# mx-mark/VideoTransformer-pytorch

Hardware: NVIDIA H100
Metric: clips/sec (BxTx3x224x224) TimeSformer-B fwd+bwd (higher is better)
Workload: dtype bf16

## Files before the change

videotransformer_pytorch_b200/csrc/vt_gemm.cu:

```cuda
#include <stdlib.h>
#include <string.h>

#include "vt_common.cuh"
#include "vt_sm90.cuh"

namespace vt {

constexpr int BM = 128;
constexpr int BK = 64;
constexpr int GEMM_THREADS = 384;
constexpr int CHUNK_BYTES = 64 * BK * 2;

struct GemmDev {
  int M, N, K;
  int kblocks, splits;
  int num_m, num_n, tiles;
  int epi;
  const float* bias;
  const float* bias2;
  void* out;
  const void* aux;
  long long ldo, ldaux;
  const int* out_row;
  const int* aux_row;
  const float* row_scale;
  long long split_stride;
  int map_period, map_skip, map_tcount;
  long long map_stride_t, map_stride_p, map_stride_b, map_base;
  float* special_out;
  long long special_ld;
  const float* a_scale;
  const float* b_scale;
};

constexpr int EPI_BOX_BYTES = 64 * 64 * 2;
constexpr int SE_F32 = 3;

template <int BN, int SE>
struct GemmCfg {
  static constexpr int A_BYTES = BM * BK * 2;
  static constexpr int B_BYTES = BN * BK * 2;
  static constexpr int STAGE_BYTES = A_BYTES + B_BYTES;
  static constexpr int EPI_TILE_BYTES = BM * BN * 2;
  static constexpr int F32_PITCH = BN + 8;
  static constexpr int EPI_BYTES = SE == SE_F32 ? BM * F32_PITCH * 4 : SE == 1 ? EPI_TILE_BYTES : 0;
  static constexpr int SMEM_LIMIT = 232448, SMEM_EXTRA = 1024  + 256 ;
  static constexpr int STAGES_FIT = (SMEM_LIMIT - SMEM_EXTRA - EPI_BYTES) / STAGE_BYTES;
  static constexpr int STAGES = STAGES_FIT < 6 ? STAGES_FIT : 6;
  static constexpr int SMEM_BYTES = STAGES * STAGE_BYTES + EPI_BYTES + SMEM_EXTRA;
  static_assert(STAGES >= 2 && SMEM_BYTES <= SMEM_LIMIT, "shared memory budget");
};

template <int BN, int TA, int TB>
__device__ __forceinline__ void wgmma_tile(float (&acc)[BN / 2], uint64_t da, uint64_t db, uint32_t scale_d) {
  if constexpr (BN == 256) wgmma_m64n256k16<TA, TB>(acc, da, db, scale_d);
  else if constexpr (BN == 192) wgmma_m64n192k16<TA, TB>(acc, da, db, scale_d);
  else wgmma_m64n128k16<TA, TB>(acc, da, db, scale_d);
}

struct EpiRow {
  char* out;
  const char* aux;
  float s;
};

__device__ __forceinline__ EpiRow epi_row(const GemmDev& p, int row, int split) {
  EpiRow r{nullptr, nullptr, 1.0f};
  if (row >= p.M) return r;
  if (p.row_scale) r.s = p.row_scale[row];
  if (p.epi == VT_EPI_F32) {
    float* out = static_cast<float*>(p.out);
    const float* aux = static_cast<const float*>(p.aux);
    if (p.map_period > 0) {
      const int outer = row / p.map_period, inner = row - outer * p.map_period;
      if (inner < p.map_skip) {
        if (p.special_out) r.out = reinterpret_cast<char*>(p.special_out + (long long)outer * p.special_ld);
        return r;
      }
      const long long off = p.map_base + (long long)(outer % p.map_tcount) * p.map_stride_t +
                            (long long)(inner - p.map_skip) * p.map_stride_p + (long long)(outer / p.map_tcount) * p.map_stride_b;
      r.out = reinterpret_cast<char*>(out + off);
      r.aux = reinterpret_cast<const char*>(aux + off);
      return r;
    }
    const int orow = p.out_row ? p.out_row[row] : row;
    if (orow >= 0) r.out = reinterpret_cast<char*>(out + (long long)split * p.split_stride + (long long)orow * p.ldo);
    if (aux) {
      const int arow = p.aux_row ? p.aux_row[row] : row;
      if (arow >= 0) r.aux = reinterpret_cast<const char*>(aux + (long long)arow * p.ldaux);
    }
    return r;
  }
  const int orow = p.out_row ? p.out_row[row] : row;
  if (orow < 0) return r;
  r.out = reinterpret_cast<char*>(static_cast<__nv_bfloat16*>(p.out) + (long long)orow * p.ldo);
  return r;
}

__device__ __forceinline__ void add_bias(const GemmDev& p, int n, float& v0, float& v1) {
  if (p.bias) {
    const float2 b = __ldg(reinterpret_cast<const float2*>(p.bias + n));
    v0 += b.x; v1 += b.y;
  }
}
__device__ __forceinline__ uint32_t gelu_pair(uint32_t z) {
  const float2 zr = unpack_bf16x2(z);
  return pack_bf16x2(gelu_fast(zr.x), gelu_fast(zr.y));
}

__device__ __forceinline__ void epi_pair(const GemmDev& p, const EpiRow& r, int n, float v0, float v1) {
  if (!r.out) return;
  add_bias(p, n, v0, v1);
  if (p.epi == VT_EPI_BF16) {
    *reinterpret_cast<uint32_t*>(reinterpret_cast<__nv_bfloat16*>(r.out) + n) = pack_bf16x2(r.s * v0, r.s * v1);
  } else if (p.epi == VT_EPI_F32) {
    float2 a = make_float2(0.f, 0.f);
    if (r.aux) a = *reinterpret_cast<const float2*>(reinterpret_cast<const float*>(r.aux) + n);
    if (p.bias2) {
      const float2 b2 = __ldg(reinterpret_cast<const float2*>(p.bias2 + n));
      a.x += b2.x; a.y += b2.y;
    }
    *reinterpret_cast<float2*>(reinterpret_cast<float*>(r.out) + n) = make_float2(fmaf(r.s, v0, a.x), fmaf(r.s, v1, a.y));
  } else {
    *reinterpret_cast<uint32_t*>(reinterpret_cast<__nv_bfloat16*>(r.out) + n) = gelu_pair(pack_bf16x2(r.s * v0, r.s * v1));
  }
}

template <int BN, int EPI>
__device__ __forceinline__ void epi_stage(const GemmDev& p, const float (&acc)[BN / 2], uint8_t* stage, int row0, int n0,
                                          int warp, int lane) {
  const int r = warp * 16 + (lane >> 2);
  float s[2] = {1.0f, 1.0f};
  if (p.row_scale) {
#pragma unroll
    for (int h = 0; h < 2; ++h)
      if (row0 + r + 8 * h < p.M) s[h] = p.row_scale[row0 + r + 8 * h];
  }
  const uint32_t a1 = smem_u32(stage) + r * 128 + 4 * (lane & 3) + ((lane >> 2) << 4);
#pragma unroll
  for (int j = 0; j < BN / 8; ++j) {
    const int n = n0 + 8 * j + 2 * (lane & 3);
    if (n >= p.N) break;
#pragma unroll
    for (int h = 0; h < 2; ++h) {
      const uint32_t off = (j >> 3) * EPI_BOX_BYTES + h * 8 * 128;
      const uint32_t o = (a1 ^ ((j & 7) << 4)) + off;
      float v0 = acc[4 * j + 2 * h], v1 = acc[4 * j + 2 * h + 1];
      add_bias(p, n, v0, v1);
      if (EPI == VT_EPI_BF16) st_shared_u32(o, pack_bf16x2(s[h] * v0, s[h] * v1));
      else st_shared_u32(o, gelu_pair(pack_bf16x2(s[h] * v0, s[h] * v1)));
    }
  }
}

struct Tile {
  int m0, n0, split, kb0, kb1;
};

template <int BN>
__device__ __forceinline__ Tile tile_at(const GemmDev& p, int t) {
  Tile c;
  const int nt = t % p.num_n, rest = t / p.num_n;
  const int mt = rest % p.num_m;
  c.split = rest / p.num_m;
  c.m0 = mt * BM;
  c.n0 = nt * BN;
  c.kb0 = (int)(((long long)p.kblocks * c.split) / p.splits);
  c.kb1 = (int)(((long long)p.kblocks * (c.split + 1)) / p.splits);
  return c;
}

template <int BN>
__device__ __forceinline__ void epi_f32_io(const GemmDev& p, float* stage, uint64_t* full, uint64_t* ready, int half, int lane) {
  constexpr int PITCH = GemmCfg<BN, SE_F32>::F32_PITCH;
  uint32_t tj = 0;
  for (int t = blockIdx.x; t < p.tiles; t += gridDim.x, ++tj) {
    const Tile c = tile_at<BN>(p, t);
    const int cols = p.N - c.n0 < BN ? p.N - c.n0 : BN;
    const uint32_t bytes = (uint32_t)cols * 4;
    const int row0 = c.m0 + half * 64 + lane;
    const EpiRow e0 = epi_row(p, row0, c.split), e1 = epi_row(p, row0 + 32, c.split);
    float* s0 = stage + lane * PITCH;
    float* s1 = s0 + 32 * PITCH;
    tma_store_wait_read_all();
    uint32_t tx = 0;
    if (p.aux) {
      if (e0.out && e0.aux) tx += bytes;
      if (e1.out && e1.aux) tx += bytes;
      for (int h = 0; h < 2; ++h) {
        const EpiRow& e = h ? e1 : e0;
        if (e.out && !e.aux)
          for (int i = 0; i < cols; i += 4) st_shared_zero16(smem_u32((h ? s1 : s0) + i));
      }
    }
    mbar_arrive_expect_tx(full, tx);
    if (tx) {
      if (e0.out && e0.aux) bulk_load_1d(s0, reinterpret_cast<const float*>(e0.aux) + c.n0, bytes, full);
      if (e1.out && e1.aux) bulk_load_1d(s1, reinterpret_cast<const float*>(e1.aux) + c.n0, bytes, full);
    }
    mbar_wait(ready, tj & 1);
    if (e0.out) bulk_store_1d(reinterpret_cast<float*>(e0.out) + c.n0, s0, bytes);
    if (e1.out) bulk_store_1d(reinterpret_cast<float*>(e1.out) + c.n0, s1, bytes);
    tma_store_commit();
  }
  tma_store_wait_read_all();
}

template <int BN>
__device__ __forceinline__ void epi_f32_stage(const GemmDev& p, const float (&acc)[BN / 2], const float* stage, int row0, int n0,
                                              int warp, int lane) {
  constexpr int PITCH = GemmCfg<BN, SE_F32>::F32_PITCH;
  const int r = warp * 16 + (lane >> 2);
  float s[2] = {1.0f, 1.0f};
  if (p.row_scale) {
#pragma unroll
    for (int h = 0; h < 2; ++h)
      if (row0 + r + 8 * h < p.M) s[h] = p.row_scale[row0 + r + 8 * h];
  }
  const uint32_t a0 = smem_u32(stage + r * PITCH + 2 * (lane & 3));
#pragma unroll
  for (int j = 0; j < BN / 8; ++j) {
    const int n = n0 + 8 * j + 2 * (lane & 3);
    if (n >= p.N) break;
#pragma unroll
    for (int h = 0; h < 2; ++h) {
      const uint32_t o = a0 + (h * 8 * PITCH + 8 * j) * 4;
      float v0 = acc[4 * j + 2 * h], v1 = acc[4 * j + 2 * h + 1];
      add_bias(p, n, v0, v1);
      float2 a = make_float2(0.f, 0.f);
      if (p.aux) a = ld_shared_f32x2(o);
      if (p.bias2) {
        const float2 b2 = __ldg(reinterpret_cast<const float2*>(p.bias2 + n));
        a.x += b2.x; a.y += b2.y;
      }
      st_shared_f32x2(o, fmaf(s[h], v0, a.x), fmaf(s[h], v1, a.y));
    }
  }
}

template <int BN, int TA, int TB, int SE, int F8>
__device__ __forceinline__ void gemm_wgmma_body(const CUtensorMap& tmA, const CUtensorMap& tmB, const CUtensorMap& tmC,
                                                const GemmDev& p) {
  using Cfg = GemmCfg<BN, SE>;
  static_assert(SE == 0 || SE == 1 || SE == SE_F32, "epilogue kinds: register, staged bf16, staged fp32");
  static_assert(!F8 || (BN == 128 && !TA && !TB), "e4m3 forms: BN = 128, K-major operands");
  static_assert(SE != SE_F32 || BN != 256, "the fp32 staging tile leaves too few ring stages at BN = 256");
  constexpr int STAGES = Cfg::STAGES;
  constexpr int KB_ELEMS = F8 ? 128 : BK;
  constexpr int HALF_BYTES = Cfg::EPI_TILE_BYTES / 2;
  extern __shared__ uint8_t smem_raw[];
  uint8_t* smem = reinterpret_cast<uint8_t*>((reinterpret_cast<uintptr_t>(smem_raw) + 1023) & ~uintptr_t(1023));
  uint8_t* epi_smem = smem + STAGES * Cfg::STAGE_BYTES;
  uint64_t* full_bar = reinterpret_cast<uint64_t*>(epi_smem + Cfg::EPI_BYTES);
  uint64_t* empty_bar = full_bar + STAGES;
  uint64_t* rows_full_bar = empty_bar + STAGES;
  uint64_t* rows_ready_bar = rows_full_bar + 2;

  const int wg = threadIdx.x >> 7;
  if (threadIdx.x == 0) {
    tma_prefetch_desc(&tmA);
    tma_prefetch_desc(&tmB);
    if (SE == 1) tma_prefetch_desc(&tmC);
    for (int i = 0; i < STAGES; ++i) {
      mbar_init(&full_bar[i], 1);
      mbar_init(&empty_bar[i], 8);
    }
    for (int h = 0; h < 2; ++h) {
      mbar_init(&rows_full_bar[h], 32);
      mbar_init(&rows_ready_bar[h], 128);
    }
    fence_barrier_init();
  }
  __syncthreads();

  if (wg == 0) {
    setmaxnreg_dec<40>();
    const int pw = threadIdx.x >> 5;
    if constexpr (SE == SE_F32) {
      if (pw == 1 || pw == 2) {
        float* rows = reinterpret_cast<float*>(epi_smem) + (pw - 1) * 64 * Cfg::F32_PITCH;
        epi_f32_io<BN>(p, rows, &rows_full_bar[pw - 1], &rows_ready_bar[pw - 1], pw - 1, threadIdx.x & 31);
      }
    }
    if (threadIdx.x == 0) {
      uint32_t it = 0;
      uint32_t tj = 0;
      for (int t = blockIdx.x; t < p.tiles; t += gridDim.x, ++tj) {
        const Tile c = tile_at<BN>(p, t);
        for (int kb = c.kb0; kb < c.kb1; ++kb, ++it) {
          const int stage = (int)(it % STAGES);
          mbar_wait(&empty_bar[stage], ((it / STAGES) & 1) ^ 1);
          uint8_t* sA = smem + stage * Cfg::STAGE_BYTES;
          uint8_t* sB = sA + Cfg::A_BYTES;
          mbar_arrive_expect_tx(&full_bar[stage], Cfg::STAGE_BYTES);
          if (!TA) {
            tma_load_2d(sA, &tmA, &full_bar[stage], kb * KB_ELEMS, c.m0);
          } else {
#pragma unroll
            for (int ch = 0; ch < BM / 64; ++ch) tma_load_2d(sA + ch * CHUNK_BYTES, &tmA, &full_bar[stage], c.m0 + ch * 64, kb * BK);
          }
          if (!TB) {
            tma_load_2d(sB, &tmB, &full_bar[stage], kb * KB_ELEMS, c.n0);
          } else {
#pragma unroll
            for (int ch = 0; ch < BN / 64; ++ch) tma_load_2d(sB + ch * CHUNK_BYTES, &tmB, &full_bar[stage], c.n0 + ch * 64, kb * BK);
          }
        }
      }
    }
    return;
  }

  setmaxnreg_inc<232>();
  const int cw = wg - 1;
  const int warp = (threadIdx.x >> 5) & 3, lane = threadIdx.x & 31;
  const bool leader = (threadIdx.x & 127) == 0;
  uint8_t* stage = epi_smem + cw * HALF_BYTES;
  uint32_t it = 0, tj = 0;
  float part[F8 ? BN / 2 : 1];
#pragma unroll
  for (int i = 0; i < (F8 ? BN / 2 : 1); ++i) part[i] = 0.f;
  for (int t = blockIdx.x; t < p.tiles; t += gridDim.x, ++tj) {
    const Tile c = tile_at<BN>(p, t);
    float acc[BN / 2];
#pragma unroll
    for (int i = 0; i < BN / 2; ++i) acc[i] = 0.f;
    if constexpr (F8) {
      for (int kb = c.kb0; kb < c.kb1; ++kb, ++it) {
        const int stage = (int)(it % STAGES);
        mbar_wait(&full_bar[stage], (it / STAGES) & 1);
        const uint32_t a_addr = smem_u32(smem + stage * Cfg::STAGE_BYTES) + cw * 64 * 128;
        const uint32_t b_addr = smem_u32(smem + stage * Cfg::STAGE_BYTES + Cfg::A_BYTES);
        wgmma_fence();
#pragma unroll
        for (int k = 0; k < 4; ++k)
          wgmma_m64n128k32_e4m3(part, sdesc_kmajor(a_addr + k * 32), sdesc_kmajor(b_addr + k * 32), k > 0 ? 1u : 0u);
        wgmma_commit();
        wgmma_wait<0>();
        if (lane == 0) mbar_arrive(&empty_bar[stage]);
#pragma unroll
        for (int i = 0; i < BN / 2; ++i) acc[i] += part[i];
      }
      const int rr = c.m0 + cw * 64 + warp * 16 + (lane >> 2);
      const float sa0 = rr < p.M ? p.a_scale[rr] : 0.f, sa1 = rr + 8 < p.M ? p.a_scale[rr + 8] : 0.f;
#pragma unroll
      for (int j = 0; j < BN / 8; ++j) {
        const int n = c.n0 + 8 * j + 2 * (lane & 3);
        if (n >= p.N) break;
        const float2 sb = __ldg(reinterpret_cast<const float2*>(p.b_scale + n));
        acc[4 * j] *= sa0 * sb.x;
        acc[4 * j + 1] *= sa0 * sb.y;
        acc[4 * j + 2] *= sa1 * sb.x;
        acc[4 * j + 3] *= sa1 * sb.y;
      }
    } else {
    int prev = -1;
    for (int kb = c.kb0; kb < c.kb1; ++kb, ++it) {
      const int stage = (int)(it % STAGES);
      mbar_wait(&full_bar[stage], (it / STAGES) & 1);
      const uint32_t a_addr = smem_u32(smem + stage * Cfg::STAGE_BYTES) + cw * (TA ? CHUNK_BYTES : 64 * 128);
      const uint32_t b_addr = smem_u32(smem + stage * Cfg::STAGE_BYTES + Cfg::A_BYTES);
      wgmma_fence();
#pragma unroll
      for (int k = 0; k < BK / 16; ++k) {
        const uint64_t da = TA ? sdesc_mnmajor(a_addr + k * 2048, CHUNK_BYTES) : sdesc_kmajor(a_addr + k * 32);
        const uint64_t db = TB ? sdesc_mnmajor(b_addr + k * 2048, CHUNK_BYTES) : sdesc_kmajor(b_addr + k * 32);
        wgmma_tile<BN, TA, TB>(acc, da, db, (kb > c.kb0 || k > 0) ? 1u : 0u);
      }
      wgmma_commit();
      wgmma_wait<1>();
      if (prev >= 0 && lane == 0) mbar_arrive(&empty_bar[prev]);
      prev = stage;
    }
    wgmma_wait<0>();
    if (lane == 0) mbar_arrive(&empty_bar[prev]);
    }

    if constexpr (SE == SE_F32) {
      const float* rows = reinterpret_cast<const float*>(epi_smem) + cw * 64 * Cfg::F32_PITCH;
      mbar_wait(&rows_full_bar[cw], tj & 1);
      epi_f32_stage<BN>(p, acc, rows, c.m0 + cw * 64, c.n0, warp, lane);
      fence_proxy_async_smem();
      mbar_arrive(&rows_ready_bar[cw]);
    } else if constexpr (SE == 1) {
      const int row0 = c.m0 + cw * 64;
      if (leader) tma_store_wait_read_all();
      named_bar_sync(1 + cw, 128);
      if (p.epi == VT_EPI_GELU_H) epi_stage<BN, VT_EPI_GELU_H>(p, acc, stage, row0, c.n0, warp, lane);
      else epi_stage<BN, VT_EPI_BF16>(p, acc, stage, row0, c.n0, warp, lane);
      fence_proxy_async_smem();
      named_bar_sync(1 + cw, 128);
      if (leader) {
        if (row0 < p.M) {
#pragma unroll
          for (int b = 0; b < BN / 64; ++b) {
            if (c.n0 + 64 * b >= p.N) break;
            tma_store_2d(&tmC, stage + b * EPI_BOX_BYTES, c.n0 + 64 * b, row0);
          }
        }
        tma_store_commit();
      }
    } else {
      const int r0 = c.m0 + cw * 64 + warp * 16 + (lane >> 2);
      const EpiRow e0 = epi_row(p, r0, c.split), e1 = epi_row(p, r0 + 8, c.split);
#pragma unroll
      for (int j = 0; j < BN / 8; ++j) {
        const int n = c.n0 + 8 * j + 2 * (lane & 3);
        if (n >= p.N) break;
        epi_pair(p, e0, n, acc[4 * j], acc[4 * j + 1]);
        epi_pair(p, e1, n, acc[4 * j + 2], acc[4 * j + 3]);
      }
    }
  }
  if (SE == 1 && leader) tma_store_wait_read_all();
}

template <int BN, int TA, int TB, int SE>
__global__ void __launch_bounds__(GEMM_THREADS, 1)
gemm_wgmma_kernel(const __grid_constant__ CUtensorMap tmA, const __grid_constant__ CUtensorMap tmB,
                  const __grid_constant__ CUtensorMap tmC, const GemmDev p) {
  gemm_wgmma_body<BN, TA, TB, SE, 0>(tmA, tmB, tmC, p);
}

template <int BN, int TA, int TB>
__global__ void __launch_bounds__(GEMM_THREADS, 1)
gemm_f32_kernel(const __grid_constant__ CUtensorMap tmA, const __grid_constant__ CUtensorMap tmB,
                const __grid_constant__ CUtensorMap tmC, const GemmDev p) {
  gemm_wgmma_body<BN, TA, TB, SE_F32, 0>(tmA, tmB, tmC, p);
}

template <int SE>
__global__ void __launch_bounds__(GEMM_THREADS, 1)
gemm_e4m3_kernel(const __grid_constant__ CUtensorMap tmA, const __grid_constant__ CUtensorMap tmB,
                 const __grid_constant__ CUtensorMap tmC, const GemmDev p) {
  gemm_wgmma_body<128, 0, 0, SE, 1>(tmA, tmB, tmC, p);
}

typedef CUresult (*EncodeTiledFn)(CUtensorMap*, CUtensorMapDataType, cuuint32_t, void*, const cuuint64_t*,
                                  const cuuint64_t*, const cuuint32_t*, const cuuint32_t*, CUtensorMapInterleave,
                                  CUtensorMapSwizzle, CUtensorMapL2promotion, CUtensorMapFloatOOBfill);

static EncodeTiledFn get_encode_fn() {
  static EncodeTiledFn fn = nullptr;
  if (!fn) {
    void* ptr = nullptr;
    cudaDriverEntryPointQueryResult qres;
    cudaError_t e = cudaGetDriverEntryPoint("cuTensorMapEncodeTiled", &ptr, cudaEnableDefault, &qres);
    if (e != cudaSuccess || qres != cudaDriverEntryPointSuccess || !ptr) return nullptr;
    fn = reinterpret_cast<EncodeTiledFn>(ptr);
  }
  return fn;
}

static int make_tmap_2d(CUtensorMap* map, int esize, const void* base, long long rows, long long cols, long long ld,
                        int box_rows) {
  EncodeTiledFn fn = get_encode_fn();
  VT_REQUIRE(fn != nullptr, "cuTensorMapEncodeTiled entry point unavailable");
  VT_REQUIRE((reinterpret_cast<uintptr_t>(base) & 15) == 0, "TMA base pointer must be 16-byte aligned");
  VT_REQUIRE((ld * esize) % 16 == 0, "TMA leading dimension must be a multiple of %d elements (got %lld)", 16 / esize, ld);
  cuuint64_t gdim[2] = {(cuuint64_t)cols, (cuuint64_t)rows};
  cuuint64_t gstr[1] = {(cuuint64_t)(ld * esize)};
  cuuint32_t box[2] = {(cuuint32_t)(128 / esize), (cuuint32_t)box_rows};
  cuuint32_t estr[2] = {1u, 1u};
  CUresult r = fn(map, esize == 2 ? CU_TENSOR_MAP_DATA_TYPE_BFLOAT16 : CU_TENSOR_MAP_DATA_TYPE_UINT8, 2, const_cast<void*>(base),
                  gdim, gstr, box, estr,
                  CU_TENSOR_MAP_INTERLEAVE_NONE, CU_TENSOR_MAP_SWIZZLE_128B, CU_TENSOR_MAP_L2_PROMOTION_L2_256B,
                  CU_TENSOR_MAP_FLOAT_OOB_FILL_NONE);
  VT_REQUIRE(r == CUDA_SUCCESS, "cuTensorMapEncodeTiled failed (%d) rows=%lld cols=%lld ld=%lld box_rows=%d", (int)r,
             rows, cols, ld, box_rows);
  return 0;
}

int make_tmap_bf16_2d(CUtensorMap* map, const void* base, long long rows, long long cols, long long ld, int box_rows) {
  return make_tmap_2d(map, 2, base, rows, cols, ld, box_rows);
}

__global__ void reduce_rows_kernel(const float* __restrict__ in, float* __restrict__ out, long long stride, int S,
                                   long long n4, int accumulate, float scale) {
  for (long long i = blockIdx.x * (long long)blockDim.x + threadIdx.x; i < n4; i += (long long)gridDim.x * blockDim.x) {
    float4 acc = make_float4(0.f, 0.f, 0.f, 0.f);
    for (int s = 0; s < S; ++s) {
      const float4 v = *reinterpret_cast<const float4*>(in + (long long)s * stride + i * 4);
      acc.x += v.x; acc.y += v.y; acc.z += v.z; acc.w += v.w;
    }
    acc.x *= scale; acc.y *= scale; acc.z *= scale; acc.w *= scale;
    float4* o = reinterpret_cast<float4*>(out + i * 4);
    if (accumulate) {
      const float4 p = *o;
      acc.x += p.x; acc.y += p.y; acc.z += p.z; acc.w += p.w;
    }
    *o = acc;
  }
}

constexpr int RT_QUADS = 4, RT_LANES = 64;
__global__ void __launch_bounds__(RT_QUADS * RT_LANES)
reduce_rows_tall_kernel(const float* __restrict__ in, float* __restrict__ out, long long stride, int S, long long n4,
                        int accumulate, float scale) {
  const int cq = threadIdx.x % RT_QUADS, rl = threadIdx.x / RT_QUADS;
  const long long i = blockIdx.x * (long long)RT_QUADS + cq;
  float4 acc = make_float4(0.f, 0.f, 0.f, 0.f);
  if (i < n4) {
    for (int s = rl; s < S; s += RT_LANES) {
      const float4 v = *reinterpret_cast<const float4*>(in + (long long)s * stride + i * 4);
      acc.x += v.x; acc.y += v.y; acc.z += v.z; acc.w += v.w;
    }
  }
  __shared__ float4 sh[RT_LANES][RT_QUADS];
  sh[rl][cq] = acc;
  __syncthreads();
  if (rl < 16) {
    float4 a = sh[rl][cq];
#pragma unroll
    for (int r = rl + 16; r < RT_LANES; r += 16) { a.x += sh[r][cq].x; a.y += sh[r][cq].y; a.z += sh[r][cq].z; a.w += sh[r][cq].w; }
    sh[rl][cq] = a;
  }
  __syncthreads();
  if (rl == 0 && i < n4) {
    float4 a = sh[0][cq];
#pragma unroll
    for (int r = 1; r < 16; ++r) { a.x += sh[r][cq].x; a.y += sh[r][cq].y; a.z += sh[r][cq].z; a.w += sh[r][cq].w; }
    a.x *= scale; a.y *= scale; a.z *= scale; a.w *= scale;
    float4* o = reinterpret_cast<float4*>(out + i * 4);
    if (accumulate) { const float4 p = *o; a.x += p.x; a.y += p.y; a.z += p.z; a.w += p.w; }
    *o = a;
  }
}

int launch_reduce_rows(const float* in, float* out, long long stride, int S, long long n, int accumulate, float scale,
                       cudaStream_t st) {
  VT_REQUIRE(n % 4 == 0 && stride % 4 == 0, "vt_reduce_rows: n and stride must be multiples of 4");
  const long long n4 = n / 4;
  if (S >= 32 && n4 <= 16 * 4096) {
    reduce_rows_tall_kernel<<<(int)((n4 + RT_QUADS - 1) / RT_QUADS), RT_QUADS * RT_LANES, 0, st>>>(in, out, stride, S, n4, accumulate, scale);
    return check_launch("reduce_rows_tall_kernel");
  }
  int blocks = (int)((n4 + 255) / 256);
  const int cap = sm_count() * 8;
  if (blocks > cap) blocks = cap;
  if (blocks < 1) blocks = 1;
  reduce_rows_kernel<<<blocks, 256, 0, st>>>(in, out, stride, S, n4, accumulate, scale);
  return check_launch("reduce_rows_kernel");
}

template <int BN, int TA, int TB, int SE, int F8 = 0>
static int launch_gemm_t(const CUtensorMap (&tm)[3], const GemmDev& d, cudaStream_t st) {
  using Cfg = GemmCfg<BN, SE>;
  void (*kernel)(const CUtensorMap, const CUtensorMap, const CUtensorMap, const GemmDev);
  if constexpr (F8) kernel = gemm_e4m3_kernel<SE>;
  else if constexpr (SE == SE_F32) kernel = gemm_f32_kernel<BN, TA, TB>;
  else kernel = gemm_wgmma_kernel<BN, TA, TB, SE>;
  static bool attr_set = false;
  if (!attr_set) {
    cudaError_t e = cudaFuncSetAttribute(kernel, cudaFuncAttributeMaxDynamicSharedMemorySize, Cfg::SMEM_BYTES);
    VT_REQUIRE(e == cudaSuccess, "cudaFuncSetAttribute(smem=%d) failed: %s", Cfg::SMEM_BYTES, cudaGetErrorString(e));
    attr_set = true;
  }
  const int grid = d.tiles < persistent_sm_count() ? d.tiles : persistent_sm_count();
  kernel<<<grid, GEMM_THREADS, Cfg::SMEM_BYTES, st>>>(tm[0], tm[1], tm[2], d);
  return check_launch(F8 ? "gemm_e4m3_kernel" : SE == SE_F32 ? "gemm_f32_kernel" : "gemm_wgmma_kernel");
}

template <int BN, int SE>
static int launch_layout(const vt_gemm_params* q, const CUtensorMap (&tm)[3], const GemmDev& d, cudaStream_t st) {
  if (!q->a_mn_major && !q->b_mn_major) return launch_gemm_t<BN, 0, 0, SE>(tm, d, st);
  if (!q->a_mn_major) return launch_gemm_t<BN, 0, 1, SE>(tm, d, st);
  if (!q->b_mn_major) return launch_gemm_t<BN, 1, 0, SE>(tm, d, st);
  return launch_gemm_t<BN, 1, 1, SE>(tm, d, st);
}

#ifndef VT_DEFAULT_STAGED_EPI
#define VT_DEFAULT_STAGED_EPI true
#endif
static int staged_kind(const vt_gemm_params* q) {
  if (!feature_on("VT_GEMM_STAGED_EPI", VT_DEFAULT_STAGED_EPI)) return 0;
  if (q->epilogue == VT_EPI_F32) {
    if (q->map_period > 0 &&
        (q->map_base % 4 || q->map_stride_t % 4 || q->map_stride_p % 4 || q->map_stride_b % 4 ||
         (q->map_special_base >= 0 && (q->map_special_base % 4 || q->map_special_stride % 4))))
      return 0;
    return SE_F32;
  }
  return q->out_row ? 0 : 1;
}

template <int BN, int F8 = 0>
static int launch_gemm(const vt_gemm_params* q, GemmDev& d, cudaStream_t st) {
  CUtensorMap tm[3];
  memset(tm, 0, sizeof(tm));
  CUtensorMap &tmA = tm[0], &tmB = tm[1];
  int rc;
  if (F8) {
    rc = make_tmap_2d(&tmA, 1, q->a, q->M, q->K, q->lda, BM);
    if (!rc) rc = make_tmap_2d(&tmB, 1, q->b, q->N, q->K, q->ldb, BN);
  } else if (!q->a_mn_major) rc = make_tmap_bf16_2d(&tmA, q->a, q->M, q->K, q->lda, BM);
  else rc = make_tmap_bf16_2d(&tmA, q->a, q->K, q->M, q->lda, BK);
  if (rc) return rc;
  if (!F8) {
    if (!q->b_mn_major) rc = make_tmap_bf16_2d(&tmB, q->b, q->N, q->K, q->ldb, BN);
    else rc = make_tmap_bf16_2d(&tmB, q->b, q->K, q->N, q->ldb, BK);
    if (rc) return rc;
  }
  d.num_m = (q->M + BM - 1) / BM;
  d.num_n = (q->N + BN - 1) / BN;
  const long long tiles = (long long)d.num_m * d.num_n * d.splits;
  VT_REQUIRE(tiles < (1LL << 31), "vt_gemm: M=%d N=%d gives too many tiles", q->M, q->N);
  d.tiles = (int)tiles;
  const long long tile_out = (long long)q->M * q->N;
  void* final_out = d.out;
  d.split_stride = 0;
  if (d.splits > 1) {
    d.out = q->workspace;
    d.ldo = q->N;
    d.split_stride = tile_out;
  }
  int se = staged_kind(q);
  if (se == SE_F32 && (BN == 256 || (d.splits > 1 && (BN != 128 || (reinterpret_cast<uintptr_t>(q->workspace) & 15))))) se = 0;
  if (se == 1) {
    rc = make_tmap_bf16_2d(&tm[2], q->out, q->M, q->N, q->ldo, 64);
    if (rc) return rc;
  }
  if constexpr (F8) {
    if (se == 1) rc = launch_gemm_t<BN, 0, 0, 1, 1>(tm, d, st);
    else if (se == SE_F32) rc = launch_gemm_t<BN, 0, 0, SE_F32, 1>(tm, d, st);
    else rc = launch_gemm_t<BN, 0, 0, 0, 1>(tm, d, st);
  } else {
    if (se == 1) rc = launch_layout<BN, 1>(q, tm, d, st);
    else if constexpr (BN != 256) {
      if (se == SE_F32) rc = launch_layout<BN, SE_F32>(q, tm, d, st);
      else rc = launch_layout<BN, 0>(q, tm, d, st);
    } else {
      rc = launch_layout<BN, 0>(q, tm, d, st);
    }
  }
  if (rc) return rc;
  if (d.splits > 1) {
    VT_REQUIRE(q->ldo == q->N, "vt_gemm: split-K requires ldo == N");
    return launch_reduce_rows(static_cast<const float*>(q->workspace), static_cast<float*>(final_out), tile_out, d.splits, tile_out,
                              0, 1.0f, st);
  }
  return 0;
}

}

static int gemm_dispatch(const vt_gemm_params* q, const float* a_scale, const float* b_scale, void* stream);

extern "C" int vt_gemm(const vt_gemm_params* q, void* stream) {
  VT_REQUIRE(q != nullptr, "vt_gemm: null params");
  return gemm_dispatch(q, nullptr, nullptr, stream);
}

extern "C" int vt_gemm_e4m3(const vt_gemm_e4m3_params* p, void* stream) {
  using namespace vt;
  VT_REQUIRE(p != nullptr, "vt_gemm_e4m3: null params");
  const vt_gemm_params* q = &p->g;
  VT_REQUIRE(p->a_scale && p->b_scale && (reinterpret_cast<uintptr_t>(p->b_scale) & 15) == 0,
             "vt_gemm_e4m3: a_scale and b_scale are required (b_scale 16-byte aligned)");
  VT_REQUIRE(!q->a_mn_major && !q->b_mn_major, "vt_gemm_e4m3: both operands must be K-major");
  VT_REQUIRE(q->K > 0 && q->K % 16 == 0 && q->lda % 16 == 0 && q->ldb % 16 == 0,
             "vt_gemm_e4m3: K, lda and ldb must be multiples of 16 (got K=%d lda=%lld ldb=%lld)", q->K, (long long)q->lda,
             (long long)q->ldb);
  VT_REQUIRE(q->force_bn == 0 || q->force_bn == 128, "vt_gemm_e4m3: the e4m3 forms run 128-wide tiles only");
  int dev = 0, major = 0;
  VT_REQUIRE(cudaGetDevice(&dev) == cudaSuccess && cudaDeviceGetAttribute(&major, cudaDevAttrComputeCapabilityMajor, dev) == cudaSuccess &&
                 major == 9, "vt_gemm_e4m3: needs an sm_90 device (compute capability %d.x found)", major);
  return gemm_dispatch(q, p->a_scale, p->b_scale, stream);
}

static int gemm_dispatch(const vt_gemm_params* q, const float* a_scale, const float* b_scale, void* stream) {
  using namespace vt;
  VT_REQUIRE(q != nullptr, "vt_gemm: null params");
  const bool f8 = a_scale != nullptr;
  VT_REQUIRE(q->M > 0 && q->N > 0 && q->K > 0, "vt_gemm: bad shape M=%d N=%d K=%d", q->M, q->N, q->K);
  VT_REQUIRE(q->N % 8 == 0, "vt_gemm: N must be a multiple of 8 (got %d)", q->N);
  VT_REQUIRE(q->a && q->b && q->out, "vt_gemm: null operand");
  VT_REQUIRE(q->epilogue == VT_EPI_BF16 || q->epilogue == VT_EPI_F32 || q->epilogue == VT_EPI_GELU_H,
             "vt_gemm: bad epilogue %d (VT_EPI_BF16 = 0, VT_EPI_F32 = 1, VT_EPI_GELU_H = 4)", q->epilogue);
  const int esz = (q->epilogue == VT_EPI_F32) ? 4 : 2;
  VT_REQUIRE((q->ldo * esz) % 16 == 0 && (reinterpret_cast<uintptr_t>(q->out) & 15) == 0,
             "vt_gemm: out must be 16B aligned with 16B-multiple row pitch");
  if (q->aux) VT_REQUIRE(q->epilogue == VT_EPI_F32, "vt_gemm: aux (the fp32 addend) needs VT_EPI_F32, got epilogue %d", q->epilogue);
  if (q->aux) VT_REQUIRE((reinterpret_cast<uintptr_t>(q->aux) & 15) == 0 && (q->ldaux * 4) % 16 == 0, "vt_gemm: aux misaligned");
  if (q->bias) VT_REQUIRE((reinterpret_cast<uintptr_t>(q->bias) & 15) == 0, "vt_gemm: bias misaligned");
  if (q->bias2) VT_REQUIRE(q->epilogue == VT_EPI_F32 && q->aux && (reinterpret_cast<uintptr_t>(q->bias2) & 15) == 0,
                           "vt_gemm: bias2 needs the fp32 epilogue with an addend, 16-byte aligned");
  VT_REQUIRE(q->force_bn == 0 || q->force_bn == 128 || q->force_bn == 192 || q->force_bn == 256,
             "vt_gemm: force_bn must be 128, 192 or 256");

  GemmDev d;
  d.M = q->M; d.N = q->N; d.K = q->K;
  d.epi = q->epilogue;
  d.bias = q->bias;
  d.bias2 = q->bias2;
  d.out = q->out; d.aux = q->aux;
  d.ldo = q->ldo; d.ldaux = q->ldaux;
  d.out_row = q->out_row; d.aux_row = q->aux_row; d.row_scale = q->row_scale;
  d.kblocks = f8 ? (q->K + 127) / 128 : (q->K + BK - 1) / BK;
  d.a_scale = a_scale; d.b_scale = b_scale;
  d.map_period = 0; d.map_skip = 0; d.map_tcount = 1;
  d.map_stride_t = d.map_stride_p = d.map_stride_b = d.map_base = 0;
  d.special_out = nullptr; d.special_ld = 0;
  if (q->map_period > 0) {
    VT_REQUIRE(q->epilogue == VT_EPI_F32 && q->aux, "vt_gemm: the affine row map applies to the fp32 residual epilogue only");
    VT_REQUIRE(q->M % q->map_period == 0 && q->map_tcount >= 1 && q->map_skip >= 0 && q->map_skip < q->map_period,
               "vt_gemm: bad affine row map (period %d, skip %d, tcount %d, M %d)", q->map_period, q->map_skip, q->map_tcount, q->M);
    VT_REQUIRE(q->map_base % 2 == 0 && q->map_stride_t % 2 == 0 && q->map_stride_p % 2 == 0 && q->map_stride_b % 2 == 0 &&
                   (q->map_special_base < 0 || (q->map_special_base % 2 == 0 && q->map_special_stride % 2 == 0)),
               "vt_gemm: affine row map offsets and strides must be even (8-byte aligned fp32 pairs)");
    d.map_period = q->map_period; d.map_skip = q->map_skip; d.map_tcount = q->map_tcount;
    d.map_stride_t = q->map_stride_t; d.map_stride_p = q->map_stride_p; d.map_stride_b = q->map_stride_b; d.map_base = q->map_base;
    d.special_out = q->map_special_base >= 0 ? static_cast<float*>(q->out) + q->map_special_base : nullptr;
    d.special_ld = q->map_special_stride;
  }

  if (f8) {
    d.splits = 1;
    return launch_gemm<128, 1>(q, d, static_cast<cudaStream_t>(stream));
  }
  const bool short_k = d.kblocks <= 16;
  const bool one_staged = staged_kind(q) == 1;
  const int sms = persistent_sm_count();
  const int num_m = (q->M + BM - 1) / BM;
  const bool can_split = q->epilogue == VT_EPI_F32 && q->workspace && !q->out_row && !q->aux && !q->row_scale && !q->bias &&
                         q->map_period == 0;
  const bool f32_staged = staged_kind(q) == SE_F32 && !can_split;
  const int cand[3] = {256, 192, 128};
  const double penalty[3] = {1.0, 1.04, 1.10};
  double best = 1e30;
  int bn = 128, splits = 1;
  for (int i = 0; i < 3; ++i) {
    if (q->force_bn && cand[i] != q->force_bn) continue;
    if (!q->force_bn && !can_split && short_k && cand[i] != 128 && !((one_staged || f32_staged) && cand[i] == 192)) continue;
    if (!q->force_bn && f32_staged && cand[i] == 256) continue;
    const int num_n = (q->N + cand[i] - 1) / cand[i];
    const int smax = can_split ? 16 : 1;
    for (int sp = 1; sp <= smax; ++sp) {
      if (sp > 1 && (d.kblocks / sp < 4 || (long long)sp * q->M * q->N * 4 > q->workspace_bytes)) break;
      const long long tiles = (long long)num_m * num_n * sp;
      const double per_cta = (double)((tiles + sms - 1) / sms);
      const double cost = per_cta * ((double)d.kblocks / sp + 8.0) * cand[i] * penalty[i];
      if (cost < best - 1e-9) { best = cost; bn = cand[i]; splits = sp; }
    }
  }
  if (can_split && q->force_splits > 0) {
    splits = q->force_splits;
    const long long max_by_ws = q->workspace_bytes / ((long long)q->M * q->N * 4);
    if (splits > max_by_ws) splits = (int)max_by_ws;
    if (splits > d.kblocks) splits = d.kblocks;
    if (splits < 1) splits = 1;
  }
  d.splits = splits;
  cudaStream_t st = static_cast<cudaStream_t>(stream);
  if (bn == 256) return launch_gemm<256>(q, d, st);
  if (bn == 192) return launch_gemm<192>(q, d, st);
  return launch_gemm<128>(q, d, st);
}

extern "C" int vt_reduce_rows(const vt_reduce_params* p, void* stream) {
  using namespace vt;
  VT_REQUIRE(p && p->in && p->out && p->S >= 1, "vt_reduce_rows: bad params");
  return launch_reduce_rows(p->in, p->out, p->stride, p->S, p->n, p->accumulate, p->scale,
                            static_cast<cudaStream_t>(stream));
}
```

Before: 276.8.

## Add stream-K work decomposition for fp32 split GEMMs with in-place fixup

Replaces the fixed split-K tile enumeration with a unit walker that supports data-parallel, even split-K, and stream-K schedules, where each persistent CTA takes a contiguous range of k-iterations across tiles. The first fragment of each tile writes straight to the output and later fragments go to workspace slots. A new fixup kernel adds them in place, replacing the separate full reduce over all split copies. Stream-K is chosen for long-K fp32 workspace GEMMs whose operands fit in L2, to cut wave quantization. The cost is an extra fixup pass and more index arithmetic, plus correctness risk in the fragment bookkeeping.

```diff
diff --git a/videotransformer_pytorch_b200/csrc/vt_gemm.cu b/videotransformer_pytorch_b200/csrc/vt_gemm.cu
--- a/videotransformer_pytorch_b200/csrc/vt_gemm.cu
+++ b/videotransformer_pytorch_b200/csrc/vt_gemm.cu
@@ -13,8 +13,9 @@
 
 struct GemmDev {
   int M, N, K;
-  int kblocks, splits;
+  int kblocks;
   int num_m, num_n, tiles;
+  int units, iters;
   int epi;
   const float* bias;
   const float* bias2;
@@ -24,7 +25,8 @@
   const int* out_row;
   const int* aux_row;
   const float* row_scale;
-  long long split_stride;
+  float* ws;
+  long long slot_stride;
   int map_period, map_skip, map_tcount;
   long long map_stride_t, map_stride_p, map_stride_b, map_base;
   float* special_out;
@@ -84,7 +86,8 @@
       return r;
     }
     const int orow = p.out_row ? p.out_row[row] : row;
-    if (orow >= 0) r.out = reinterpret_cast<char*>(out + (long long)split * p.split_stride + (long long)orow * p.ldo);
+    if (split) r.out = reinterpret_cast<char*>(p.ws + (long long)(split - 1) * p.slot_stride + (long long)row * p.N);
+    else if (orow >= 0) r.out = reinterpret_cast<char*>(out + (long long)orow * p.ldo);
     if (aux) {
       const int arow = p.aux_row ? p.aux_row[row] : row;
       if (arow >= 0) r.aux = reinterpret_cast<const char*>(aux + (long long)arow * p.ldaux);
@@ -157,16 +160,57 @@
   int m0, n0, split, kb0, kb1;
 };
 
+__host__ __device__ __forceinline__ int unit_begin(int u, int iters, int units) {
+  return (int)((long long)u * iters / units);
+}
+__host__ __device__ __forceinline__ int unit_of(int x, int iters, int units) { return ((x + 1) * units - 1) / iters; }
+
+struct Walk {
+  int u, pos, end;
+};
+
+__device__ __forceinline__ Walk walk_begin(const GemmDev& p) {
+  Walk w;
+  w.u = blockIdx.x;
+  w.pos = w.end = 0;
+  if (p.units % p.tiles) {
+    w.pos = unit_begin(w.u, p.iters, p.units);
+    w.end = unit_begin(w.u + 1, p.iters, p.units);
+  }
+  return w;
+}
+
 template <int BN>
-__device__ __forceinline__ Tile tile_at(const GemmDev& p, int t) {
+__device__ __forceinline__ Tile walk_take(const GemmDev& p, Walk& w) {
   Tile c;
-  const int nt = t % p.num_n, rest = t / p.num_n;
-  const int mt = rest % p.num_m;
-  c.split = rest / p.num_m;
-  c.m0 = mt * BM;
-  c.n0 = nt * BN;
-  c.kb0 = (int)(((long long)p.kblocks * c.split) / p.splits);
-  c.kb1 = (int)(((long long)p.kblocks * (c.split + 1)) / p.splits);
+  int t;
+  if (p.units == p.tiles) {
+    t = w.u;
+    c.kb0 = 0;
+    c.kb1 = p.kblocks;
+    c.split = 0;
+    w.u += gridDim.x;
+  } else if (p.units % p.tiles == 0) {
+    const int s = p.units / p.tiles;
+    t = w.u % p.tiles;
+    c.split = w.u / p.tiles;
+    c.kb0 = c.split * p.kblocks / s;
+    c.kb1 = (c.split + 1) * p.kblocks / s;
+    w.u += gridDim.x;
+  } else {
+    t = w.pos / p.kblocks;
+    c.kb0 = w.pos - t * p.kblocks;
+    c.kb1 = min(p.kblocks, c.kb0 + (w.end - w.pos));
+    c.split = c.kb0 ? w.u - unit_of(t * p.kblocks, p.iters, p.units) : 0;
+    w.pos += c.kb1 - c.kb0;
+    if (w.pos == w.end) {
+      w.u += gridDim.x;
+      w.pos = unit_begin(w.u, p.iters, p.units);
+      w.end = unit_begin(w.u + 1, p.iters, p.units);
+    }
+  }
+  c.m0 = (t / p.num_n) * BM;
+  c.n0 = (t % p.num_n) * BN;
   return c;
 }
 
@@ -174,8 +218,8 @@
 __device__ __forceinline__ void epi_f32_io(const GemmDev& p, float* stage, uint64_t* full, uint64_t* ready, int half, int lane) {
   constexpr int PITCH = GemmCfg<BN, SE_F32>::F32_PITCH;
   uint32_t tj = 0;
-  for (int t = blockIdx.x; t < p.tiles; t += gridDim.x, ++tj) {
-    const Tile c = tile_at<BN>(p, t);
+  for (Walk w = walk_begin(p); w.u < p.units; ++tj) {
+    const Tile c = walk_take<BN>(p, w);
     const int cols = p.N - c.n0 < BN ? p.N - c.n0 : BN;
     const uint32_t bytes = (uint32_t)cols * 4;
     const int row0 = c.m0 + half * 64 + lane;
@@ -284,9 +328,8 @@
     }
     if (threadIdx.x == 0) {
       uint32_t it = 0;
-      uint32_t tj = 0;
-      for (int t = blockIdx.x; t < p.tiles; t += gridDim.x, ++tj) {
-        const Tile c = tile_at<BN>(p, t);
+      for (Walk w = walk_begin(p); w.u < p.units;) {
+        const Tile c = walk_take<BN>(p, w);
         for (int kb = c.kb0; kb < c.kb1; ++kb, ++it) {
           const int stage = (int)(it % STAGES);
           mbar_wait(&empty_bar[stage], ((it / STAGES) & 1) ^ 1);
@@ -320,8 +363,8 @@
   float part[F8 ? BN / 2 : 1];
 #pragma unroll
   for (int i = 0; i < (F8 ? BN / 2 : 1); ++i) part[i] = 0.f;
-  for (int t = blockIdx.x; t < p.tiles; t += gridDim.x, ++tj) {
-    const Tile c = tile_at<BN>(p, t);
+  for (Walk w = walk_begin(p); w.u < p.units; ++tj) {
+    const Tile c = walk_take<BN>(p, w);
     float acc[BN / 2];
 #pragma unroll
     for (int i = 0; i < BN / 2; ++i) acc[i] = 0.f;
@@ -543,6 +586,25 @@
   return check_launch("reduce_rows_kernel");
 }
 
+template <int BN>
+__global__ void streamk_fixup_kernel(const GemmDev p) {
+  const int col = 4 * (blockIdx.x * blockDim.x + threadIdx.x);
+  if (col >= p.N) return;
+  for (int row = blockIdx.y; row < p.M; row += gridDim.y) {
+    const int it0 = ((row / BM) * p.num_n + col / BN) * p.kblocks;
+    const int frags = unit_of(it0 + p.kblocks - 1, p.iters, p.units) - unit_of(it0, p.iters, p.units) + 1;
+    if (frags == 1) continue;
+    float4* o = reinterpret_cast<float4*>(static_cast<float*>(p.out) + (long long)row * p.ldo + col);
+    float4 acc = *o;
+    const float* slot = p.ws + (long long)row * p.N + col;
+    for (int f = 1; f < frags; ++f, slot += p.slot_stride) {
+      const float4 v = *reinterpret_cast<const float4*>(slot);
+      acc.x += v.x; acc.y += v.y; acc.z += v.z; acc.w += v.w;
+    }
+    *o = acc;
+  }
+}
+
 template <int BN, int TA, int TB, int SE, int F8 = 0>
 static int launch_gemm_t(const CUtensorMap (&tm)[3], const GemmDev& d, cudaStream_t st) {
   using Cfg = GemmCfg<BN, SE>;
@@ -556,7 +618,7 @@
     VT_REQUIRE(e == cudaSuccess, "cudaFuncSetAttribute(smem=%d) failed: %s", Cfg::SMEM_BYTES, cudaGetErrorString(e));
     attr_set = true;
   }
-  const int grid = d.tiles < persistent_sm_count() ? d.tiles : persistent_sm_count();
+  const int grid = d.units < persistent_sm_count() ? d.units : persistent_sm_count();
   kernel<<<grid, GEMM_THREADS, Cfg::SMEM_BYTES, st>>>(tm[0], tm[1], tm[2], d);
   return check_launch(F8 ? "gemm_e4m3_kernel" : SE == SE_F32 ? "gemm_f32_kernel" : "gemm_wgmma_kernel");
 }
@@ -585,7 +647,7 @@
 }
 
 template <int BN, int F8 = 0>
-static int launch_gemm(const vt_gemm_params* q, GemmDev& d, cudaStream_t st) {
+static int launch_gemm(const vt_gemm_params* q, GemmDev& d, int units, cudaStream_t st) {
   CUtensorMap tm[3];
   memset(tm, 0, sizeof(tm));
   CUtensorMap &tmA = tm[0], &tmB = tm[1];
@@ -603,19 +665,23 @@
   }
   d.num_m = (q->M + BM - 1) / BM;
   d.num_n = (q->N + BN - 1) / BN;
-  const long long tiles = (long long)d.num_m * d.num_n * d.splits;
+  const long long tiles = (long long)d.num_m * d.num_n;
   VT_REQUIRE(tiles < (1LL << 31), "vt_gemm: M=%d N=%d gives too many tiles", q->M, q->N);
   d.tiles = (int)tiles;
-  const long long tile_out = (long long)q->M * q->N;
-  void* final_out = d.out;
-  d.split_stride = 0;
-  if (d.splits > 1) {
-    d.out = q->workspace;
-    d.ldo = q->N;
-    d.split_stride = tile_out;
+  d.units = units ? units : d.tiles;
+  const bool split = d.units != d.tiles;
+  d.iters = 0;
+  d.ws = nullptr;
+  d.slot_stride = (long long)q->M * q->N;
+  if (split) {
+    const long long iters = tiles * d.kblocks;
+    VT_REQUIRE(q->workspace && d.units <= iters && (iters + 1) * d.units < (1LL << 31),
+               "vt_gemm: split plan of %d units over %lld iterations", d.units, iters);
+    d.iters = (int)iters;
+    d.ws = static_cast<float*>(q->workspace);
   }
   int se = staged_kind(q);
-  if (se == SE_F32 && (BN == 256 || (d.splits > 1 && (BN != 128 || (reinterpret_cast<uintptr_t>(q->workspace) & 15))))) se = 0;
+  if (se == SE_F32 && (BN == 256 || (split && (BN != 128 || (reinterpret_cast<uintptr_t>(q->workspace) & 15))))) se = 0;
   if (se == 1) {
     rc = make_tmap_bf16_2d(&tm[2], q->out, q->M, q->N, q->ldo, 64);
     if (rc) return rc;
@@ -633,13 +699,38 @@
       rc = launch_layout<BN, 0>(q, tm, d, st);
     }
   }
-  if (rc) return rc;
-  if (d.splits > 1) {
-    VT_REQUIRE(q->ldo == q->N, "vt_gemm: split-K requires ldo == N");
-    return launch_reduce_rows(static_cast<const float*>(q->workspace), static_cast<float*>(final_out), tile_out, d.splits, tile_out,
-                              0, 1.0f, st);
-  }
-  return 0;
+  if (rc || !split) return rc;
+  const dim3 grid((q->N / 4 + 127) / 128, q->M < 65535 ? q->M : 65535);
+  streamk_fixup_kernel<BN><<<grid, 128, 0, st>>>(d);
+  return check_launch("streamk_fixup_kernel");
+}
+
+constexpr int MAX_FRAGMENTS = 16;
+
+static int streamk_units(const vt_gemm_params* q, int kblocks, int sms) {
+  const long long tiles = (long long)((q->M + BM - 1) / BM) * ((q->N + 127) / 128), iters = tiles * kblocks;
+  const int units = sms;
+  if (units <= tiles || units > iters || (iters + 1) * units >= (1LL << 31)) return 0;
+  int max_frags = 1;
+  for (int t = 0; t < (int)tiles; ++t) {
+    const int f = unit_of((t + 1) * kblocks - 1, (int)iters, units) - unit_of(t * kblocks, (int)iters, units) + 1;
+    max_frags = f > max_frags ? f : max_frags;
+  }
+  if (max_frags > MAX_FRAGMENTS || (long long)(max_frags - 1) * q->M * q->N * 4 > q->workspace_bytes) return 0;
+  return units;
+}
+
+static long long l2_bytes() {
+  static long long cached[64] = {0};
+  int dev = 0;
+  cudaGetDevice(&dev);
+  if (dev < 0 || dev >= 64) dev = 0;
+  if (cached[dev] == 0) {
+    int n = 0;
+    if (cudaDeviceGetAttribute(&n, cudaDevAttrL2CacheSize, dev) != cudaSuccess || n <= 0) n = 50 << 20;
+    cached[dev] = n;
+  }
+  return cached[dev];
 }
 
 }
@@ -714,10 +805,8 @@
     d.special_ld = q->map_special_stride;
   }
 
-  if (f8) {
-    d.splits = 1;
-    return launch_gemm<128, 1>(q, d, static_cast<cudaStream_t>(stream));
-  }
+  cudaStream_t st = static_cast<cudaStream_t>(stream);
+  if (f8) return launch_gemm<128, 1>(q, d, 0, st);
   const bool short_k = d.kblocks <= 16;
   const bool one_staged = staged_kind(q) == 1;
   const int sms = persistent_sm_count();
@@ -725,6 +814,11 @@
   const bool can_split = q->epilogue == VT_EPI_F32 && q->workspace && !q->out_row && !q->aux && !q->row_scale && !q->bias &&
                          q->map_period == 0;
   const bool f32_staged = staged_kind(q) == SE_F32 && !can_split;
+  if (can_split && !q->force_bn && !q->force_splits && d.kblocks >= 64 &&
+      (long long)(q->M + q->N) * q->K * 2 <= l2_bytes()) {
+    const int units = streamk_units(q, d.kblocks, sms);
+    if (units) return launch_gemm<128>(q, d, units, st);
+  }
   const int cand[3] = {256, 192, 128};
   const double penalty[3] = {1.0, 1.04, 1.10};
   double best = 1e30;
@@ -734,7 +828,7 @@
     if (!q->force_bn && !can_split && short_k && cand[i] != 128 && !((one_staged || f32_staged) && cand[i] == 192)) continue;
     if (!q->force_bn && f32_staged && cand[i] == 256) continue;
     const int num_n = (q->N + cand[i] - 1) / cand[i];
-    const int smax = can_split ? 16 : 1;
+    const int smax = can_split ? MAX_FRAGMENTS : 1;
     for (int sp = 1; sp <= smax; ++sp) {
       if (sp > 1 && (d.kblocks / sp < 4 || (long long)sp * q->M * q->N * 4 > q->workspace_bytes)) break;
       const long long tiles = (long long)num_m * num_n * sp;
@@ -748,13 +842,13 @@
     const long long max_by_ws = q->workspace_bytes / ((long long)q->M * q->N * 4);
     if (splits > max_by_ws) splits = (int)max_by_ws;
     if (splits > d.kblocks) splits = d.kblocks;
+    if (splits > MAX_FRAGMENTS) splits = MAX_FRAGMENTS;
     if (splits < 1) splits = 1;
   }
-  d.splits = splits;
-  cudaStream_t st = static_cast<cudaStream_t>(stream);
-  if (bn == 256) return launch_gemm<256>(q, d, st);
-  if (bn == 192) return launch_gemm<192>(q, d, st);
-  return launch_gemm<128>(q, d, st);
+  const int units = splits > 1 ? num_m * ((q->N + bn - 1) / bn) * splits : 0;
+  if (bn == 256) return launch_gemm<256>(q, d, units, st);
+  if (bn == 192) return launch_gemm<192>(q, d, units, st);
+  return launch_gemm<128>(q, d, units, st);
 }
 
 extern "C" int vt_reduce_rows(const vt_reduce_params* p, void* stream) {
```

After: 281.7 (median of 6 runs). 1.7% higher.
